# davidesantangelo/krep

Measured on NVIDIA H100. Metric: GB/s scanned (HBM-resident corpus), higher is better.
Workload: dtype u8

## Files before the change

### krep_b200/csrc/engine.cu

```cuda
#include <cub/device/device_radix_sort.cuh>
#include <algorithm>
#include <chrono>
#include <cstdarg>
#include <cstdio>
#include <cstdlib>
#include <cstring>
#include <mutex>
#include <thread>
#include "common.h"
#include "corpus.h"
#include "engine.h"

namespace kb {

static thread_local int t_err = 0;
static thread_local char t_errmsg[512] = "";

void set_error(int code, const char *fmt, ...)
{
    t_err = code;
    va_list ap;
    va_start(ap, fmt);
    vsnprintf(t_errmsg, sizeof t_errmsg, fmt, ap);
    va_end(ap);
// ... 397 lines not shown
    for (size_t i = 1; i < m; i++)
    {
        int k = pi[i - 1];
        while (k > 0 && ch(i) != ch((size_t)k)) k = pi[(size_t)k - 1];
        if (ch(i) == ch((size_t)k)) k++;
        pi[i] = k;
    }
    return pi[m - 1] == 0;
}

Plan *regex_plan_build(const search_params_t *P, std::string *why)
{
    std::string re;
    if (!regex_source(P, &re))
    {
        *why = "no pattern";
        return nullptr;
    }
    RegexDfa *D = new RegexDfa();
    if (regex_compile(re, !P->case_sensitive, D, why) != 0)
    {
        delete D;
        return nullptr;
    }
    Plan *pl = new Plan();
    pl->algo = KREP_B200_ALGO_REGEX;
    pl->is_regex = true;
    pl->case_sensitive = P->case_sensitive;
    pl->whole_word = P->whole_word ? 1 : 0;
    pl->regex = re;
    pl->rx = D;
    pl->filter_name = D->widened ? "regex-lines-widened" : "regex-lines";
    std::lock_guard<std::mutex> lp(g_plans_mu);
    g_all_plans.push_back(pl);
    return pl;
}

Plan *plan_build(const search_params_t *P, int algo, bool only_matching)
{
    if (!P) return nullptr;
    if (algo == KREP_B200_ALGO_REGEX)
    {
        std::string why;
        Plan *pl = regex_plan_build(P, &why);
        if (!pl) set_error(-3, "this regex is not run on the GPU (%s); use the host's regex_search", why.c_str());
        return pl;
    }
    Plan *pl = new Plan();
    pl->algo = algo;
    pl->case_sensitive = P->case_sensitive;
    pl->count_lines = P->count_lines_mode;
    if (algo == KREP_B200_ALGO_AC)
    {
        pl->is_ac = true;
        if (P->num_patterns > AC_MAX_PATTERNS)
        {
            set_error(-3, "too many patterns (%zu > %u)", (size_t)P->num_patterns, AC_MAX_PATTERNS);
            delete pl;
            return nullptr;
        }
        for (size_t k = 0; k < P->num_patterns; k++)
        {
            const size_t len = P->pattern_lens[k];
            if (len > 1024)
            {
                set_error(-3, "pattern %zu longer than 1024 bytes (krep.c:77)", k);
                delete pl;
                return nullptr;
            }
            pl->patterns.emplace_back(P->patterns[k] ? P->patterns[k] : "", len);
            pl->pat_lens.push_back((uint32_t)len);
        }
        pl->whole_word = P->whole_word ? 1 : 0;
        if (ac_build_tables(pl) != 0)
        {
            delete pl;
            return nullptr;
        }
        std::lock_guard<std::mutex> lp(g_plans_mu);
        g_all_plans.push_back(pl);
        return pl;
    }
    size_t m = P->pattern_len;
    if (algo == KREP_B200_ALGO_MEMCHR) m = m ? 1 : 0;
    if (m == 0 || m > 1024 || !P->pattern)
    {
        set_error(-3, "literal plan needs 1..1024 pattern bytes (got %zu)", m);
        delete pl;
        return nullptr;
    }
    pl->pattern.assign(P->pattern, m);
    pl->m = (uint32_t)m;
    pl->emit_len = (algo == KREP_B200_ALGO_MEMCHR_SHORT && only_matching) ? 1u : (uint32_t)m;
    pl->border_free = border_free(pl->pattern, pl->case_sensitive);
    pl->built_only_matching = only_matching;
    if (P->whole_word)
    {
        bool tag = pl->emit_len != pl->m;
        if (algo == KREP_B200_ALGO_AVX2 || algo == KREP_B200_ALGO_AVX512 || algo == KREP_B200_ALGO_NEON) tag = true;
        if (!tag && !pl->border_free)
            tag = algo == KREP_B200_ALGO_KMP || (algo == KREP_B200_ALGO_SSE42 && !only_matching);
        pl->whole_word = tag ? 2 : 1;
    }
    pl->h_val.resize(m);
    pl->h_msk.resize(m);
    const uint8_t *pb = (const uint8_t *)pl->pattern.data();
    for (size_t k = 0; k < m; k++)
    {
        pl->h_msk[k] = (!pl->case_sensitive && is_alpha_c(pb[k])) ? 0xDF : 0xFF;
        pl->h_val[k] = pb[k] & pl->h_msk[k];
    }
    pl->fold = pl->case_sensitive ? 0xFFFFFFFFu : 0xDFDFDFDFu;
    if (pl->emit_len >= 7)
    {
        pl->filter = FILTER_ALIGNED4;
        for (int d = 0; d < 4; d++) pl->K[d] = le32(pb + d, 4) & pl->fold;
        pl->win_mask = 0xFFFFFFFFu;
        pl->filter_name = pl->case_sensitive ? "aligned4" : "aligned4-fold";
    }
    else
    {
        pl->filter = FILTER_WINDOW4;
        const uint32_t wl = pl->emit_len < 4 ? pl->emit_len : 4;
        pl->win_mask = wl == 4 ? 0xFFFFFFFFu : ((1u << (8 * wl)) - 1);
        pl->K[0] = le32(pb, wl) & pl->fold & pl->win_mask;
        pl->filter_name = pl->case_sensitive ? "window4" : "window4-fold";
    }
    std::lock_guard<std::mutex> lp(g_plans_mu);
    g_all_plans.push_back(pl);
    return pl;
}

int launch_scan(DevCtx &E, const Plan *plan, const krep_b200_shard_t *sh, int want_positions, cudaStream_t stream, int slot,
                unsigned long long *regex_lines, bool regex_matches)
{
    if (((uintptr_t)sh->d_text & 15) != 0)
    {
        set_error(-3, "shard text pointer must be 16-byte aligned");
        return -3;
    }
    const PlanDev *pd = plan_on_device(plan, E);
    if (!pd) return -2;
    uint64_t own_end = sh->own_end < sh->avail_len ? sh->own_end : sh->avail_len;
    if (plan->is_regex)
    {
        if (regex_matches && (!plan->rx->offsets_exact || !want_positions))
        {
            set_error(-3, "regex match mode needs an offsets_exact plan and the occurrence list");
            return -3;
        }
        if (regex_matches && sh->global_offset + sh->avail_len >= REGEX_MATCH_MAX_OFFSET)
        {
            set_error(-3, "regex match offsets must stay below 2^48 bytes of global offset (key layout, csrc/common.h)");
            return -3;
        }
        RegexLaunch a;
        a.text = (const uint8_t *)sh->d_text;
        a.avail_len = sh->avail_len;
        a.own_begin = sh->own_begin;
        a.own_end = own_end;
        a.global_offset = sh->global_offset;
        a.prev_byte = sh->prev_byte;
        a.next_byte = sh->next_byte;
        a.trans = pd->d_regex;
        a.ntrans = (uint32_t)plan->rx->trans.size();
        a.nclasses = plan->rx->nclasses;
        a.start = plan->rx->start;
        a.nl_class = plan->rx->nl_class;
        a.out = E.d_list[slot];
        a.cap = want_positions ? E.key_cap : 0;
        a.counter = slot_counter(E, slot);
        a.line_count = regex_lines;
        a.matches = regex_matches ? 1u : 0u;
        a.nmtrans = (uint32_t)plan->rx->match.size();
        a.match_bol = plan->rx->match_bol;
        a.match_mid = plan->rx->match_mid;
        launch_regex(a, E.sm_count, stream);
        return 0;
    }
    if (plan->is_ac)
    {
        if (sh->global_offset + sh->avail_len >= (1ull << 40))
        {
            set_error(-3, "pattern-set shards must end below 2^40 bytes of global offset (key layout, csrc/common.h)");
            return -3;
        }
        AcLaunch a;
        a.text = (const uint8_t *)sh->d_text;
        a.avail_len = sh->avail_len;
        a.own_begin = sh->own_begin;
        a.own_end = own_end;
        a.global_offset = sh->global_offset;
        a.prev_byte = sh->prev_byte;
        a.next_byte = sh->next_byte;
        a.out = E.d_list[slot];
        a.cap = want_positions ? E.key_cap : 0;
        a.counter = slot_counter(E, slot);
        a.whole_word = plan->whole_word;
        a.want_positions = (uint32_t)want_positions;
        launch_ac(plan, pd->ac, a, E.sm_count, stream);
        return 0;
    }
    LitDevParams p;
    memset(&p, 0, sizeof p);
    p.text = (const uint8_t *)sh->d_text;
    p.avail_len = sh->avail_len;
    p.own_begin = sh->own_begin;
    p.own_end = own_end;
    p.global_offset = sh->global_offset;
    p.prev_byte = sh->prev_byte;
    p.next_byte = sh->next_byte;
    uint64_t total_groups;
    if (plan->filter == FILTER_ALIGNED4)
    {
        total_groups = sh->avail_len / 16;
        p.tail_start = total_groups ? total_groups * 16 - 3 : 0;
    }
    else
    {
        total_groups = sh->avail_len >= 20 ? (sh->avail_len - 20) / 16 + 1 : 0;
        p.tail_start = total_groups * 16;
    }
    p.group_begin = sh->own_begin / 16;
    p.group_end = (own_end + 2) / 16 + 1;
    if (p.group_end > total_groups) p.group_end = total_groups;
    if (p.group_begin > p.group_end) p.group_begin = p.group_end;
    p.m = plan->m;
    p.emit_len = plan->emit_len;
    for (int d = 0; d < 4; d++) p.K[d] = plan->K[d];
    p.fold = plan->fold;
    p.win_mask = plan->win_mask;
    p.mulc[0] = 1u << 24;
    p.mulc[1] = 1u << 16;
    p.mulc[2] = 1u << 8;
    p.pat_val = pd->d_pat_val;
    p.pat_mask = pd->d_pat_mask;
    p.out = E.d_list[slot];
    p.cap = want_positions ? E.key_cap : 0;
    p.counter = slot_counter(E, slot);
    p.whole_word = plan->whole_word;
    p.want_positions = (uint32_t)want_positions;
    launch_literal(plan, p, E.sm_count, stream);
    return 0;
}

int reset_counter(DevCtx &E, int slot, cudaStream_t stream)
{
    if (E.counter_clean[slot]) return 0;
    CK(cudaMemsetAsync(slot_counter(E, slot), 0, 64, stream));
    E.counter_clean[slot] = true;
    return 0;
}

static constexpr int FIN_THREADS = 512, FIN_SLICES = 16, FIN_KEYS = FIN_THREADS / FIN_SLICES, FIN_PIECE = 2048;

__global__ void __launch_bounds__(FIN_THREADS) k_finish(unsigned long long *counter, const uint64_t *__restrict__ keys, uint64_t cap,
                                                        uint64_t *d_pack, int want_sort)
{
    __shared__ uint64_t s_keys[FIN_PIECE];
    __shared__ unsigned long long s_cnt;
    if (threadIdx.x == 0) s_cnt = counter[0];
    __syncthreads();
    const unsigned long long cnt = s_cnt;
    if (blockIdx.x == 0 && threadIdx.x == 0) d_pack[0] = cnt;
    const bool sorting = want_sort && cnt != 0 && cnt <= PACK_KEYS && cnt <= cap;
    const uint32_t n = sorting ? (uint32_t)cnt : 0u;
    const uint32_t idx = blockIdx.x * FIN_KEYS + threadIdx.x / FIN_SLICES, slice = threadIdx.x % FIN_SLICES;
    if (blockIdx.x * FIN_KEYS < n)
    {
        const uint64_t mine = idx < n ? keys[idx] : ~0ull;
        uint32_t rank = 0;
        for (uint32_t base = 0; base < n; base += FIN_PIECE)
        {
            const uint32_t m = n - base < FIN_PIECE ? n - base : FIN_PIECE;
            for (uint32_t j = threadIdx.x; j < FIN_PIECE; j += FIN_THREADS) s_keys[j] = j < m ? keys[base + j] : ~0ull;
            __syncthreads();
            const uint32_t mr = (m + 63u) & ~63u;
#pragma unroll 8
            for (uint32_t j = slice; j < mr; j += FIN_SLICES) rank += s_keys[j] < mine ? 1u : 0u;
            __syncthreads();
        }
#pragma unroll
        for (int o = 1; o < FIN_SLICES; o <<= 1) rank += __shfl_xor_sync(0xffffffffu, rank, o);
        if (idx < n && slice == 0) d_pack[1 + rank] = mine;
    }
    __syncthreads();
    if (threadIdx.x == 0)
    {
        __threadfence();
        const unsigned long long done = atomicAdd(&counter[1], 1ULL);
        if (done == gridDim.x - 1)
        {
            counter[0] = 0;
            counter[1] = 0;
        }
    }
}

int finish_scan(DevCtx &E, int slot, int want_sort, cudaStream_t stream)
{
    k_finish<<<PACK_KEYS / FIN_KEYS, FIN_THREADS, 0, stream>>>(slot_counter(E, slot), E.d_list[slot], E.key_cap, E.d_pack[slot],
                                                                 (want_sort && E.d_list[slot]) ? 1 : 0);
    CK(cudaGetLastError());
    CK(cudaMemcpyAsync(E.h_pack[slot], E.d_pack[slot], (want_sort ? PACK_KEYS + 1 : 1) * sizeof(uint64_t), cudaMemcpyDeviceToHost, stream));
    CK(cudaEventRecord(E.ev_done[slot], stream));
    count_launch();
    E.counter_clean[slot] = true;
    return 0;
}

int sort_keys(DevCtx &E, int slot, uint64_t n, int end_bit, cudaStream_t stream, const uint64_t **sorted)
{
    *sorted = E.d_list[slot];
    if (n < 2) return 0;
    cub::DoubleBuffer<uint64_t> db(E.d_list[slot], E.d_alt);
    size_t need = 0;
    CK(cub::DeviceRadixSort::SortKeys(nullptr, need, db, (int64_t)n, 0, end_bit, stream));
    if (need > E.sort_tmp_bytes)
    {
        CK(cudaStreamSynchronize(stream));
        cudaFree(E.d_sort_tmp);
        E.d_sort_tmp = nullptr;
        E.sort_tmp_bytes = 0;
        CK(cudaMalloc(&E.d_sort_tmp, need));
        E.sort_tmp_bytes = need;
    }
    CK(cub::DeviceRadixSort::SortKeys(E.d_sort_tmp, need, db, (int64_t)n, 0, end_bit, stream));
    *sorted = db.Current();
    return 0;
}

static int bits_for(uint64_t v)
{
    int b = 1;
    while (b < 64 && (v >> b)) b++;
    return b;
}

int key_end_bit(const Plan *plan, uint64_t max_offset, bool regex_matches)
{
    const int shift = plan->is_ac ? AC_END_SHIFT : regex_matches ? REGEX_MATCH_SHIFT : LIT_TAG_BITS;
    int b = bits_for(max_offset) + shift;
    return b > 64 ? 64 : b;
}

__global__ void __launch_bounds__(256) k_line_bounds(const uint8_t *__restrict__ text, uint64_t avail, uint64_t go,
                                                     const uint64_t *__restrict__ keys, uint64_t n, int is_ac, int has_prev,
                                                     int has_next, uint64_t *__restrict__ out)
{
    const uint64_t i = ((uint64_t)blockIdx.x * blockDim.x + threadIdx.x) >> 5;
    const int lane = threadIdx.x & 31;
    if (i >= n) return;
    auto start_of = [&](uint64_t key) -> uint64_t {
        if (!is_ac) return (key >> LIT_TAG_BITS) - go;
        return (key >> AC_END_SHIFT) - (1024 - ((key >> AC_LEN_SHIFT) & 1023)) - go;
    };
    const uint64_t s = start_of(keys[i]);
    const uint64_t lb = (!is_ac && i > 0) ? start_of(keys[i - 1]) : 0;
    const uint64_t ub = (!is_ac && i + 1 < n) ? start_of(keys[i + 1]) : avail;
    uint64_t ls = (!is_ac && i > 0) ? LB_SAME_AS_PREV : (has_prev ? LB_OUTSIDE_SHARD : go);
    for (uint64_t hi = s; hi > lb;)
    {
        const uint64_t w0 = hi >= lb + 128 ? hi - 128 : lb;
        int best = -1;
#pragma unroll
        for (int k = 0; k < 4; k++)
        {
            const uint64_t p = w0 + (uint64_t)lane * 4 + k;
            if (p < hi && text[p] == '\n') best = lane * 4 + k;
        }
        best = __reduce_max_sync(0xffffffffu, best);
        if (best >= 0)
        {
            ls = go + w0 + (uint64_t)best + 1;
            break;
        }
        hi = w0;
    }
    uint64_t le = (!is_ac && i + 1 < n) ? LB_SAME_AS_NEXT : (has_next ? LB_OUTSIDE_SHARD : go + avail);
    for (uint64_t lo = s; lo < ub; lo += 128)
    {
        int best = 1 << 20;
#pragma unroll
        for (int k = 3; k >= 0; k--)
        {
            const uint64_t p = lo + (uint64_t)lane * 4 + k;
            if (p < ub && text[p] == '\n') best = lane * 4 + k;
        }
        best = __reduce_min_sync(0xffffffffu, best);
        if (best < (1 << 20))
        {
            le = go + lo + (uint64_t)best;
            break;
        }
    }
    if (lane == 0)
    {
        out[2 * i] = ls;
        out[2 * i + 1] = le;
    }
}

static int line_bounds(DevCtx &E, const Plan *plan, const krep_b200_shard_t *sh, const uint64_t *d_sorted, uint64_t n,
                       cudaStream_t stream, const uint64_t **d_bounds)
{
    *d_bounds = nullptr;
    if (n == 0) return 0;
    if (2 * n > E.bounds_cap)
    {
        CK(cudaStreamSynchronize(stream));
        cudaFree(E.d_bounds);
        E.d_bounds = nullptr;
        E.bounds_cap = 0;
        const uint64_t cap = 2 * n + n / 4 + 1024;
        CK(cudaMalloc(&E.d_bounds, cap * sizeof(uint64_t)));
        E.bounds_cap = cap;
    }
    const uint64_t threads = n * 32;
    const int has_prev = sh->prev_byte >= 0 && sh->prev_byte != '\n';
    const int has_next = sh->next_byte >= 0 && sh->next_byte != '\n';
    k_line_bounds<<<(unsigned)((threads + 255) / 256), 256, 0, stream>>>((const uint8_t *)sh->d_text, sh->avail_len, sh->global_offset,
                                                                        d_sorted, n, plan->is_ac ? 1 : 0, has_prev, has_next, E.d_bounds);
    CK(cudaGetLastError());
    count_launch();
    *d_bounds = E.d_bounds;
    return 0;
}

int scan_begin(DevCtx &E, const Plan *plan, const krep_b200_shard_t *sh, int want_positions, cudaStream_t stream, int *slot_out)
{
    if (!stream) stream = E.scan_stream;
    if (want_positions && ensure_keys(E, 1) != 0) return -2;
    const int slot = E.next_slot;
    if (E.pend[slot].active)
    {
        set_error(-3, "krep_b200_scan_shard_begin: %d scans are already in flight on device %d", SCAN_SLOTS, E.device);
        return -3;
    }
    CK(cudaStreamWaitEvent(stream, E.ev_done[slot], 0));
    if (reset_counter(E, slot, stream) != 0) return -2;
    CK(cudaEventRecord(E.ev_a[slot], stream));
    int rc = launch_scan(E, plan, sh, want_positions, stream, slot);
    if (rc != 0) return rc;
    CK(cudaEventRecord(E.ev_b[slot], stream));
    CK(cudaGetLastError());
    if (finish_scan(E, slot, want_positions, stream) != 0) return -2;
    PendingScan &P = E.pend[slot];
    P.active = true;
    P.plan = plan;
    P.shard = *sh;
    P.want_positions = want_positions;
    P.stream = stream;
    E.next_slot = (slot + 1) % SCAN_SLOTS;
    *slot_out = slot;
    return 0;
}

int scan_end(DevCtx &E, int slot, ScanOut *out)
{
    PendingScan &P = E.pend[slot];
    if (slot < 0 || slot >= SCAN_SLOTS || !P.active)
    {
        set_error(-3, "krep_b200_scan_shard_end: no scan in flight in slot %d", slot);
        return -3;
    }
    P.active = false;
    const Plan *plan = P.plan;
    const krep_b200_shard_t *sh = &P.shard;
    cudaStream_t stream = P.stream;
    reset_kernel_ms();
    for (int attempt = 0; attempt < 3; attempt++)
    {
        CK(cudaEventSynchronize(E.ev_done[slot]));
        const uint64_t cnt = E.h_pack[slot][0];
        float ms = 0.f;
        cudaEventElapsedTime(&ms, E.ev_a[slot], E.ev_b[slot]);
        add_kernel_ms(ms);
        *out = ScanOut();
        out->count = cnt;
        out->device = E.device;
        out->serial = ++E.serial;
        E.result_stream = stream;
        if (!P.want_positions) return 0;
        if (cnt <= E.key_cap)
        {
            int rc = 0;
            out->stored = cnt;
            if (cnt <= PACK_KEYS)
            {
                out->d_keys = E.d_pack[slot] + 1;
                out->h_sorted = E.h_pack[slot] + 1;
            }
            else
                rc = sort_keys(E, slot, cnt, key_end_bit(plan, sh->global_offset + sh->avail_len), stream, &out->d_keys);
            if (rc == 0 && plan->count_lines) rc = line_bounds(E, plan, sh, out->d_keys, cnt, stream, &out->d_bounds);
            return rc;
        }
        out->overflow = 1;
        for (int s2 = 0; s2 < SCAN_SLOTS; s2++)
            if (s2 != slot && E.pend[s2].active)
            {
                set_error(-3, "krep_b200_scan_shard_end: the occurrence list overflowed while another scan is in flight; end each "
                              "scan before beginning the next until the list has grown");
                return -3;
            }
        if (ensure_keys(E, cnt + cnt / 8 + 1024) != 0) return -2;
        if (reset_counter(E, slot, stream) != 0) return -2;
        CK(cudaEventRecord(E.ev_a[slot], stream));
        int rc = launch_scan(E, plan, sh, 1, stream, slot);
        if (rc != 0) return rc;
        CK(cudaEventRecord(E.ev_b[slot], stream));
        if (finish_scan(E, slot, 1, stream) != 0) return -2;
    }
    set_error(-4, "occurrence list kept overflowing");
    return -4;
}

int scan_shard(DevCtx &E, const Plan *plan, const krep_b200_shard_t *sh, int want_positions, cudaStream_t stream, ScanOut *out)
{
    int slot = 0;
    int rc = scan_begin(E, plan, sh, want_positions, stream, &slot);
    if (rc != 0) return rc;
    return scan_end(E, slot, out);
}

int fetch_keys(DevCtx &E, const ScanOut &so, const uint64_t **h)
{
    *h = nullptr;
    if (so.stored == 0) return 0;
    if (so.h_sorted)
    {
        *h = so.h_sorted;
        return 0;
    }
    if (so.stored > E.h_keys_cap)
    {
        cudaFreeHost(E.h_keys);
        E.h_keys = nullptr;
        E.h_keys_cap = 0;
        uint64_t cap = so.stored + so.stored / 4;
        if (cap < (1u << 16)) cap = 1u << 16;
        CK(cudaMallocHost(&E.h_keys, cap * sizeof(uint64_t)));
        E.h_keys_cap = cap;
    }
    cudaStream_t s = E.result_stream ? E.result_stream : E.scan_stream;
    CK(cudaMemcpyAsync(E.h_keys, so.d_keys, so.stored * sizeof(uint64_t), cudaMemcpyDeviceToHost, s));
    CK(cudaStreamSynchronize(s));
    *h = E.h_keys;
    return 0;
}

uint64_t merge_key_lists(const uint64_t *const *lists, const uint64_t *counts, uint32_t n_lists, uint64_t *dst)
{
    uint64_t total = 0;
    std::vector<uint64_t> cut;
    for (uint32_t i = 0; i < n_lists; i++)
    {
        if (counts[i] == 0) continue;
        if (dst + total != lists[i]) memmove(dst + total, lists[i], counts[i] * sizeof(uint64_t));
        cut.push_back(total);
        total += counts[i];
    }
    for (size_t i = 1; i < cut.size(); i++)
        if (dst[cut[i] - 1] > dst[cut[i]]) std::inplace_merge(dst, dst + cut[i], dst + (i + 1 < cut.size() ? cut[i + 1] : total));
    return total;
}

__global__ void __launch_bounds__(256) k_corpus(const __grid_constant__ CorpusParams c, uint8_t *dst, uint64_t global_offset,
                                                uint64_t len)
{
    const uint64_t groups = (len + 15) / 16;
    for (uint64_t g = (uint64_t)blockIdx.x * blockDim.x + threadIdx.x; g < groups; g += (uint64_t)gridDim.x * blockDim.x)
    {
        alignas(16) uint8_t b[16];
        corpus_fill16(c, global_offset + g * 16, b);
        const uint64_t off = g * 16;
        if (off + 16 <= len && (((uintptr_t)(dst + off)) & 15) == 0)
            *reinterpret_cast<uint4 *>(dst + off) = *reinterpret_cast<const uint4 *>(b);
        else
            for (int k = 0; k < 16 && off + k < len; k++) dst[off + k] = b[k];
    }
}

static int corpus_params(const krep_b200_corpus_spec_t *spec, CorpusParams *c)
{
    memset(c, 0, sizeof *c);
    c->seed = spec->seed;
    c->plant_seed = spec->plant_seed;
    c->plant_period = spec->plant_period;
    c->needle_len = spec->needle_len;
    c->flags = spec->flags;
    if (spec->needle_len > 64)
    {
        set_error(-3, "corpus needle longer than 64 bytes");
        return -3;
    }
    if (spec->plant_period && (spec->plant_period % 16 != 0 || spec->plant_period < 4ull * spec->needle_len + 32))
    {
        set_error(-3, "corpus plant_period must be a multiple of 16 and >= 4*needle_len+32");
        return -3;
    }
    if (spec->needle_len) memcpy(c->needle, spec->needle, spec->needle_len);
    return 0;
}

}

using namespace kb;

extern "C" {

int krep_b200_init(int device)
{
    g_keep_visible = true;
    warm_join();
    std::lock_guard<std::recursive_mutex> lk(engine_mutex());
    clear_error();
    if (visible_devices() == 0)
    {
        set_error(-1, "no CUDA device available; this engine has no CPU fallback");
        return -1;
    }
    if (device < 0)
    {
        device = primary_device();
        if (device < 0) return -1;
    }
    if (!ctx_get(device)) return krep_b200_last_error() ? krep_b200_last_error() : -1;
    g_primary = device;
    return 0;
}
void krep_b200_shutdown(void) { engine_shutdown(); }
int krep_b200_last_error(void) { return t_err; }
const char *krep_b200_last_error_string(void) { return t_errmsg; }
const char *krep_b200_version(void) { return "krep_b200 0.2.0 (sm_90a)"; }
int krep_b200_device_count(void)
{
    warm_join();
    return visible_devices();
}
void krep_b200_warmup(void) { warm_start(); }

float krep_b200_last_kernel_ms(void) { return t_kernel_ms; }
uint64_t krep_b200_launch_count(void) { return g_launches; }
void krep_b200_reset_launch_count(void) { g_launches = 0; }

krep_b200_plan_t *krep_b200_plan_create(const search_params_t *params, int algo)
{
    warm_join();
    std::lock_guard<std::recursive_mutex> lk(engine_mutex());
    clear_error();
    if (!params) return nullptr;
    if (visible_devices() == 0)
    {
        set_error(-1, "no CUDA device available; this engine has no CPU fallback");
        return nullptr;
    }
    return reinterpret_cast<krep_b200_plan_t *>(plan_build(params, resolve_algo(params, algo), krep_b200_get_only_matching()));
}
void krep_b200_plan_destroy(krep_b200_plan_t *plan)
{
    std::lock_guard<std::recursive_mutex> lk(engine_mutex());
    plan_free(reinterpret_cast<Plan *>(plan));
}
const char *krep_b200_plan_filter_name(const krep_b200_plan_t *plan)
{
    return plan ? reinterpret_cast<const Plan *>(plan)->filter_name.c_str() : "";
}

static DevCtx *ctx_of_pointer(const void *d_ptr)
{
    cudaPointerAttributes a;
    if (cudaPointerGetAttributes(&a, d_ptr) == cudaSuccess && a.type == cudaMemoryTypeDevice) return ctx_get(a.device);
    cudaGetLastError();
    return ctx_primary();
}

static void fill_result(const ScanOut &so, const krep_b200_shard_t *shard, int slot, krep_b200_device_result_t *out)
{
    out->count = so.count;
    out->stored = so.stored;
    out->d_keys = so.d_keys;
    out->overflow = so.overflow;
    out->text_len = shard->global_offset + shard->avail_len;
    out->d_line_bounds = so.d_bounds;
    out->device = so.device;
    out->slot = slot;
    out->serial = so.serial;
}

int krep_b200_scan_shard_begin(const krep_b200_plan_t *plan, const krep_b200_shard_t *shard, int want_positions, void *stream,
                               int *ticket)
{
    std::lock_guard<std::recursive_mutex> lk(engine_mutex());
    clear_error();
    if (!plan || !shard || !ticket)
    {
        set_error(-3, "krep_b200_scan_shard_begin: null argument");
        return -3;
    }
    DeviceGuard guard;
    DevCtx *C = ctx_of_pointer(shard->d_text);
    if (!C) return -1;
    int slot = 0;
    int rc = scan_begin(*C, reinterpret_cast<const Plan *>(plan), shard, want_positions, (cudaStream_t)stream, &slot);
    *ticket = C->device * SCAN_SLOTS + slot;
    return rc;
}

int krep_b200_scan_shard_end(int ticket, krep_b200_device_result_t *out)
{
    std::lock_guard<std::recursive_mutex> lk(engine_mutex());
    clear_error();
    if (!out || ticket < 0 || ticket >= MAX_DEV * SCAN_SLOTS)
    {
        set_error(-3, "krep_b200_scan_shard_end: bad argument");
        return -3;
    }
    DeviceGuard guard;
    DevCtx *C = ctx_get(ticket / SCAN_SLOTS);
    if (!C) return -1;
    const int slot = ticket % SCAN_SLOTS;
    const krep_b200_shard_t shard = C->pend[slot].shard;
    ScanOut so;
    int rc = scan_end(*C, slot, &so);
    fill_result(so, &shard, slot, out);
    return rc;
}

int krep_b200_scan_shard(const krep_b200_plan_t *plan, const krep_b200_shard_t *shard, int want_positions,
                         void *stream, krep_b200_device_result_t *out)
{
    int ticket = 0;
    int rc = krep_b200_scan_shard_begin(plan, shard, want_positions, stream, &ticket);
    if (rc != 0) return rc;
    if (!out)
    {
        set_error(-3, "krep_b200_scan_shard: null argument");
        return -3;
    }
    return krep_b200_scan_shard_end(ticket, out);
}

}

int kb::regex_scan_keys(DevCtx &E, const Plan *plan, const krep_b200_shard_t *shard, int mode, const char *who, uint64_t *cnt_out,
                        const uint64_t **d_sorted, uint64_t *device_lines)
{
    for (int s = 0; s < SCAN_SLOTS; s++)
        if (E.pend[s].active)
        {
            set_error(-3, "%s: a scan is in flight on device %d", who, E.device);
            return -3;
        }
    if (ensure_keys(E, 1) != 0 || (mode == 1 && ensure_line_out(E, 1) != 0)) return -2;
    unsigned long long *d_lines = mode == 1 ? (unsigned long long *)E.d_line_out : nullptr;
    const int slot = 0;
    cudaStream_t st = E.scan_stream;
    ++E.serial;
    for (int attempt = 0; attempt < 3; attempt++)
    {
        CK(cudaStreamWaitEvent(st, E.ev_done[slot], 0));
        if (reset_counter(E, slot, st) != 0) return -2;
        if (d_lines) CK(cudaMemsetAsync(d_lines, 0, sizeof(unsigned long long), st));
        int rc = launch_scan(E, plan, shard, 1, st, slot, d_lines, mode == 2);
        if (rc != 0) return rc;
        if (finish_scan(E, slot, 1, st) != 0) return -2;
        if (d_lines) CK(cudaMemcpyAsync(E.h_line_out, d_lines, sizeof(uint64_t), cudaMemcpyDeviceToHost, st));
        CK(cudaStreamSynchronize(st));
        const uint64_t cnt = E.h_pack[slot][0];
        if (cnt > E.key_cap)
        {
            if (ensure_keys(E, cnt + cnt / 8 + 1024) != 0) return -2;
            continue;
        }
        *d_sorted = E.d_pack[slot] + 1;
        if (cnt > PACK_KEYS)
        {
            rc = sort_keys(E, slot, cnt, key_end_bit(plan, shard->global_offset + shard->avail_len, mode == 2), st, d_sorted);
            if (rc != 0) return rc;
        }
        *cnt_out = cnt;
        if (device_lines) *device_lines = d_lines ? E.h_line_out[0] : 0;
        return 0;
    }
    set_error(-4, "occurrence list kept overflowing");
    return -4;
}

extern "C" {

int64_t krep_b200_regex_scan_shard_raw(const krep_b200_plan_t *plan_, const krep_b200_shard_t *shard, int mode, uint64_t *keys,
                                       uint64_t cap, uint64_t *device_lines)
{
    std::lock_guard<std::recursive_mutex> lk(engine_mutex());
    clear_error();
    const Plan *plan = reinterpret_cast<const Plan *>(plan_);
    if (!plan || !shard || (cap && !keys))
    {
        set_error(-3, "krep_b200_regex_scan_shard_raw: null argument");
        return -3;
    }
    if (!plan->is_regex || mode < 0 || mode > 2 || (mode == 1 && !plan->rx->count_exact) || (mode == 2 && !plan->rx->offsets_exact))
    {
        set_error(-3, "krep_b200_regex_scan_shard_raw: mode %d is not available for this plan", mode);
        return -3;
    }
    DeviceGuard guard;
    DevCtx *Cp = ctx_of_pointer(shard->d_text);
    if (!Cp) return -1;
    DevCtx &E = *Cp;
    uint64_t cnt = 0;
    const uint64_t *d_sorted = nullptr;
    const int rc = regex_scan_keys(E, plan, shard, mode, "krep_b200_regex_scan_shard_raw", &cnt, &d_sorted, device_lines);
    if (rc != 0) return rc;
    const uint64_t n = cnt < cap ? cnt : cap;
    if (cnt <= PACK_KEYS)
    {
        if (n) memcpy(keys, E.h_pack[0] + 1, n * sizeof(uint64_t));
    }
    else if (n)
    {
        CK(cudaMemcpyAsync(keys, d_sorted, n * sizeof(uint64_t), cudaMemcpyDeviceToHost, E.scan_stream));
        CK(cudaStreamSynchronize(E.scan_stream));
    }
    return (int64_t)cnt;
}

int krep_b200_export_keys(const krep_b200_device_result_t *dev, void *d_dst, uint64_t max_keys, void *stream)
{
    std::lock_guard<std::recursive_mutex> lk(engine_mutex());
    clear_error();
    if (!dev || !d_dst) return -3;
    const uint64_t n = dev->stored < max_keys ? dev->stored : max_keys;
    if (n == 0) return 0;
    DeviceGuard guard;
    DevCtx *C = ctx_get(dev->device);
    if (!C) return -1;
    cudaStream_t s = stream ? (cudaStream_t)stream : (C->result_stream ? C->result_stream : C->scan_stream);
    CK(cudaMemcpyAsync(d_dst, dev->d_keys, n * sizeof(uint64_t), cudaMemcpyDeviceToDevice, s));
    if (!stream) CK(cudaStreamSynchronize(s));
    return 0;
}

int krep_b200_export_packed(const krep_b200_device_result_t *dev, void *d_dst, uint64_t max_keys, void *stream)
{
    std::lock_guard<std::recursive_mutex> lk(engine_mutex());
    clear_error();
    if (!dev || !d_dst) return -3;
    DeviceGuard guard;
    DevCtx *C = ctx_get(dev->device);
    if (!C) return -1;
    cudaStream_t s = stream ? (cudaStream_t)stream : (C->result_stream ? C->result_stream : C->scan_stream);
    const uint64_t n = dev->stored < max_keys ? dev->stored : max_keys;
    if (dev->serial == C->serial && dev->stored <= PACK_KEYS && dev->slot >= 0 && dev->slot < SCAN_SLOTS)
        CK(cudaMemcpyAsync(d_dst, C->d_pack[dev->slot], (n + 1) * sizeof(uint64_t), cudaMemcpyDeviceToDevice, s));
    else
    {
        CK(cudaMemcpyAsync(d_dst, C->d_pack[dev->slot & (SCAN_SLOTS - 1)], sizeof(uint64_t), cudaMemcpyDeviceToDevice, s));
        if (n) CK(cudaMemcpyAsync((uint64_t *)d_dst + 1, dev->d_keys, n * sizeof(uint64_t), cudaMemcpyDeviceToDevice, s));
    }
    if (!stream) CK(cudaStreamSynchronize(s));
    return 0;
}

int krep_b200_export_packed_async(int ticket, void *d_dst, uint64_t max_keys)
{
    std::lock_guard<std::recursive_mutex> lk(engine_mutex());
    clear_error();
    if (!d_dst || ticket < 0 || ticket >= MAX_DEV * SCAN_SLOTS || max_keys > PACK_KEYS)
    {
        set_error(-3, "krep_b200_export_packed_async: bad argument");
        return -3;
    }
    DeviceGuard guard;
    DevCtx *C = ctx_get(ticket / SCAN_SLOTS);
    if (!C) return -1;
    const int slot = ticket % SCAN_SLOTS;
    if (!C->pend[slot].active)
    {
        set_error(-3, "krep_b200_export_packed_async: no scan in flight for this ticket");
        return -3;
    }
    cudaStream_t s = C->pend[slot].stream;
    CK(cudaStreamWaitEvent(s, C->ev_done[slot], 0));
    CK(cudaMemcpyAsync(d_dst, C->d_pack[slot], (max_keys + 1) * sizeof(uint64_t), cudaMemcpyDeviceToDevice, s));
    return 0;
}

uint64_t krep_b200_merge_keys(const uint64_t *const *lists, const uint64_t *counts, uint32_t n_lists, uint64_t *dst)
{
    if (!lists || !counts || !dst) return 0;
    return merge_key_lists(lists, counts, n_lists, dst);
}

uint64_t krep_b200_ac_key_end(uint64_t key) { return key >> AC_END_SHIFT; }
uint64_t krep_b200_ac_key_start(uint64_t key)
{
    const uint64_t len = 1024 - ((key >> AC_LEN_SHIFT) & 1023);
    return (key >> AC_END_SHIFT) - len;
}
uint32_t krep_b200_ac_key_pattern(uint64_t key) { return (uint32_t)(key & (AC_MAX_PATTERNS - 1)); }

int krep_b200_corpus_generate(const krep_b200_corpus_spec_t *spec, void *d_dst, uint64_t global_offset, uint64_t len,
                              void *stream)
{
    std::lock_guard<std::recursive_mutex> lk(engine_mutex());
    clear_error();
    DeviceGuard guard;
    DevCtx *C = ctx_of_pointer(d_dst);
    if (!C) return -1;
    CorpusParams c;
    if (corpus_params(spec, &c) != 0) return -3;
    if (global_offset % 16 != 0)
    {
        set_error(-3, "corpus global_offset must be a multiple of 16");
        return -3;
    }
    if (len == 0) return 0;
    cudaStream_t s = stream ? (cudaStream_t)stream : C->scan_stream;
    const uint64_t groups = (len + 15) / 16;
    uint64_t blocks = (groups + 255) / 256;
    const uint64_t maxb = (uint64_t)C->sm_count * 16;
    if (blocks > maxb) blocks = maxb;
    k_corpus<<<(unsigned)blocks, 256, 0, s>>>(c, (uint8_t *)d_dst, global_offset, len);
    CK(cudaGetLastError());
    if (!stream) CK(cudaStreamSynchronize(s));
    return 0;
}

int krep_b200_corpus_generate_host(const krep_b200_corpus_spec_t *spec, void *dst, uint64_t global_offset, uint64_t len)
{
    CorpusParams c;
    if (corpus_params(spec, &c) != 0) return -3;
    uint8_t *o = (uint8_t *)dst;
    uint64_t i = global_offset, end = global_offset + len;
    while (i < end)
    {
        const uint64_t g0 = i & ~15ull;
        uint8_t b[16];
        corpus_fill16(c, g0, b);
        for (uint64_t k = i - g0; k < 16 && g0 + k < end; k++) o[g0 + k - global_offset] = b[k];
        i = g0 + 16;
    }
    return 0;
}

}
```

### krep_b200/csrc/scan_literal.cu

```cuda
#include <mutex>
#include "common.h"
#include "lit_filters.cuh"

#ifndef KREP_B200_WARP_EMIT
#define KREP_B200_WARP_EMIT 1
#endif

namespace kb {

__device__ __noinline__ unsigned verify_emit(const LitDevParams &p, long long cand)
{
    const unsigned tag = verify_exact(p, cand);
    if (!tag) return 0;
    if (p.want_positions)
    {
        const unsigned long long slot = atomicAdd(p.counter, 1ULL);
        if (slot < p.cap) p.out[slot] = ((p.global_offset + (uint64_t)cand) << LIT_TAG_BITS) | (tag & 7u);
        return 0;
    }
    return 1;
}

__device__ __noinline__ unsigned slow_aligned4(const LitDevParams &p, uint64_t group, uint4 v)
{
    unsigned n = 0;
    const uint32_t w[4] = {v.x & p.fold, v.y & p.fold, v.z & p.fold, v.w & p.fold};
#pragma unroll
    for (int k = 0; k < 4; k++)
#pragma unroll
        for (int d = 0; d < 4; d++)
            if (w[k] == p.K[d]) n += verify_emit(p, (long long)(group * 16 + 4 * k) - d);
    return n;
}

template <bool WINDOW>
__device__ __noinline__ unsigned emit_warp(const LitDevParams &p, uint64_t group, uint4 v, uint32_t nx, bool mine)
{
    const uint32_t lane = threadIdx.x & 31;
    uint32_t valid = 0;
    uint64_t tags = 0;
    if (mine)
    {
        const uint32_t w[5] = {v.x, v.y, v.z, v.w, nx};
        if (WINDOW)
        {
            const uint32_t mask = p.fold & p.win_mask, k0 = p.K[0];
#pragma unroll
            for (int k = 0; k < 4; k++)
#pragma unroll
                for (int r = 0; r < 4; r++)
                {
                    const uint32_t win = r == 0 ? w[k] : __funnelshift_r(w[k], w[k + 1], 8 * r);
                    if ((win & mask) == k0)
                    {
                        const unsigned t = verify_exact(p, (long long)(group * 16 + 4 * k + r));
                        if (t)
                        {
                            valid |= 1u << (4 * k + r);
                            tags |= (uint64_t)(t & 7u) << (3 * (4 * k + r));
                        }
                    }
                }
        }
        else
        {
#pragma unroll
            for (int k = 0; k < 4; k++)
#pragma unroll
                for (int d = 0; d < 4; d++)
                    if ((w[k] & p.fold) == p.K[d])
                    {
                        const unsigned t = verify_exact(p, (long long)(group * 16 + 4 * k) - d);
                        if (t)
                        {
                            valid |= 1u << (4 * k + d);
                            tags |= (uint64_t)(t & 7u) << (3 * (4 * k + d));
                        }
                    }
        }
    }
    const uint32_t n = (uint32_t)__popc(valid);
    if (!p.want_positions) return n;
    uint32_t incl = n;
#pragma unroll
    for (int o = 1; o < 32; o <<= 1)
    {
        const uint32_t t = __shfl_up_sync(0xffffffffu, incl, o);
        if (lane >= (uint32_t)o) incl += t;
    }
    const uint32_t total = __shfl_sync(0xffffffffu, incl, 31);
    if (total == 0) return 0;
    unsigned long long base = 0;
    if (lane == 31) base = atomicAdd(p.counter, (unsigned long long)total);
    base = __shfl_sync(0xffffffffu, base, 31);
    unsigned long long slot = base + (incl - n);
    while (valid)
    {
        const uint32_t i = (uint32_t)__ffs(valid) - 1;
        valid &= valid - 1;
        const long long start = WINDOW ? (long long)(group * 16 + i) : (long long)(group * 16 + (i & ~3u)) - (long long)(i & 3u);
        if (slot < p.cap) p.out[slot] = ((p.global_offset + (uint64_t)start) << LIT_TAG_BITS) | ((tags >> (3 * i)) & 7u);
        slot++;
    }
    return 0;
}

__device__ __forceinline__ void tail_and_count(const LitDevParams &p, unsigned long long local_cnt)
{
    if (blockIdx.x == 0 && threadIdx.x < 32 && p.avail_len >= p.emit_len)
    {
        const uint64_t last = p.avail_len - p.emit_len;
        for (uint64_t s = p.tail_start + threadIdx.x; s <= last; s += 32) local_cnt += verify_emit(p, (long long)s);
    }
    if (!p.want_positions)
    {
#pragma unroll
        for (int o = 16; o > 0; o >>= 1) local_cnt += __shfl_xor_sync(0xffffffffu, local_cnt, o);
        if ((threadIdx.x & 31) == 0 && local_cnt) atomicAdd(p.counter, local_cnt);
    }
}

template <bool FOLD, int UNROLL>
__global__ void __launch_bounds__(256, 4) k_lit_aligned4(const __grid_constant__ LitDevParams p)
{
    const uint4 *__restrict__ t4 = reinterpret_cast<const uint4 *>(p.text);
    const uint32_t k0 = p.K[0], k1 = p.K[1], k2 = p.K[2], k3 = p.K[3], fold = p.fold;
    unsigned long long local_cnt = 0;
    const uint64_t tile = (uint64_t)blockDim.x * UNROLL;
    const uint64_t stride = (uint64_t)gridDim.x * tile;
    uint64_t g0 = p.group_begin + (uint64_t)blockIdx.x * tile;
    for (; g0 + tile <= p.group_end; g0 += stride)
    {
        uint4 v[UNROLL];
#pragma unroll
        for (int u = 0; u < UNROLL; u++) v[u] = ld_stream(t4 + g0 + (uint64_t)u * blockDim.x + threadIdx.x);
        bool hit = false;
#pragma unroll
        for (int u = 0; u < UNROLL; u++) hit |= hit_vec<FOLD>(v[u], fold, k0, k1, k2, k3);
#if KREP_B200_WARP_EMIT
        if (__any_sync(0xffffffffu, hit))
        {
#pragma unroll
            for (int u = 0; u < UNROLL; u++)
            {
                const bool mine = hit_vec<FOLD>(v[u], fold, k0, k1, k2, k3);
                if (__any_sync(0xffffffffu, mine))
                    local_cnt += emit_warp<false>(p, g0 + (uint64_t)u * blockDim.x + threadIdx.x, v[u], 0u, mine);
            }
        }
#else
        if (hit)
        {
#pragma unroll
            for (int u = 0; u < UNROLL; u++)
                if (hit_vec<FOLD>(v[u], fold, k0, k1, k2, k3))
                    local_cnt += slow_aligned4(p, g0 + (uint64_t)u * blockDim.x + threadIdx.x, v[u]);
        }
#endif
    }
    if (g0 < p.group_end)
    {
        for (int u = 0; u < UNROLL; u++)
        {
            const uint64_t g = g0 + (uint64_t)u * blockDim.x + threadIdx.x;
            if (g < p.group_end)
            {
                const uint4 v = ld_stream(t4 + g);
                if (hit_vec<FOLD>(v, fold, k0, k1, k2, k3)) local_cnt += slow_aligned4(p, g, v);
            }
        }
    }
    tail_and_count(p, local_cnt);
}

__device__ __noinline__ unsigned slow_window4(const LitDevParams &p, uint64_t group, uint4 v, uint32_t nx)
{
    unsigned n = 0;
    const uint32_t w[5] = {v.x, v.y, v.z, v.w, nx};
    const uint32_t mask = p.fold & p.win_mask, k0 = p.K[0];
#pragma unroll
    for (int k = 0; k < 4; k++)
#pragma unroll
        for (int r = 0; r < 4; r++)
        {
            const uint32_t win = r == 0 ? w[k] : __funnelshift_r(w[k], w[k + 1], 8 * r);
            if ((win & mask) == k0) n += verify_emit(p, (long long)(group * 16 + 4 * k + r));
        }
    return n;
}

#ifndef KREP_B200_W4_NX
#define KREP_B200_W4_NX 2
#endif
#ifndef KREP_B200_W4_WARP_EMIT
#define KREP_B200_W4_WARP_EMIT 0
#endif
#ifdef KREP_B200_W4_CS
#define WLOAD(q) ld_stream(q)
#else
#define WLOAD(q) __ldg(q)
#endif
template <bool FOLD, bool MASKED, int UNROLL>
__global__ void __launch_bounds__(256, 4) k_lit_window4(const __grid_constant__ LitDevParams p)
{
    const uint4 *__restrict__ t4 = reinterpret_cast<const uint4 *>(p.text);
    const uint32_t fold = p.fold, mask = p.win_mask, k0 = p.K[0];
    const uint32_t c1 = p.mulc[0], c2 = p.mulc[1], c3 = p.mulc[2];
    const bool lane31 = (threadIdx.x & 31) == 31;
    unsigned long long local_cnt = 0;
    const uint64_t tile = (uint64_t)blockDim.x * UNROLL;
    const uint64_t stride = (uint64_t)gridDim.x * tile;
    uint64_t g0 = p.group_begin + (uint64_t)blockIdx.x * tile;
    for (; g0 + tile <= p.group_end; g0 += stride)
    {
        uint4 v[UNROLL];
        uint32_t nx[UNROLL];
#pragma unroll
        for (int u = 0; u < UNROLL; u++)
        {
            const uint4 *q = t4 + g0 + (uint64_t)u * blockDim.x + threadIdx.x;
            v[u] = WLOAD(q);
#if KREP_B200_W4_NX == 0
            nx[u] = __ldg(reinterpret_cast<const uint32_t *>(q + 1));
#elif KREP_B200_W4_NX == 2
            nx[u] = 0u;
            asm volatile("{\n\t.reg .pred p;\n\tsetp.ne.u32 p, %2, 0;\n\t@p ld.global.nc.u32 %0, [%1];\n\t}"
                         : "+r"(nx[u])
                         : "l"(reinterpret_cast<const uint32_t *>(q + 1)), "r"((uint32_t)lane31));
#else
            nx[u] = lane31 ? __ldg(reinterpret_cast<const uint32_t *>(q + 1)) : 0u;
#endif
        }
#if KREP_B200_W4_NX != 0
#pragma unroll
        for (int u = 0; u < UNROLL; u++)
        {
            const uint32_t nb = __shfl_down_sync(0xffffffffu, v[u].x, 1);
#if KREP_B200_W4_NX == 2
            nx[u] = lane31 ? nx[u] : nb;
#else
            if (!lane31) nx[u] = nb;
#endif
        }
#endif
        uint32_t hm = 0;
#pragma unroll
        for (int u = 0; u < UNROLL; u++)
            hm |= hit_vec_w<FOLD, MASKED>(v[u], nx[u], fold, mask, k0, c1, c2, c3) ? (1u << u) : 0u;
        if constexpr (MASKED || KREP_B200_W4_WARP_EMIT)
        {
            const uint32_t anyhm = __reduce_or_sync(0xffffffffu, hm);
            if (anyhm)
            {
#pragma unroll
                for (int u = 0; u < UNROLL; u++)
                    if ((anyhm >> u) & 1u)
                        local_cnt += emit_warp<true>(p, g0 + (uint64_t)u * blockDim.x + threadIdx.x, v[u], nx[u], (hm >> u) & 1u);
            }
        }
        else if (hm)
        {
#pragma unroll
            for (int u = 0; u < UNROLL; u++)
                if ((hm >> u) & 1u) local_cnt += slow_window4(p, g0 + (uint64_t)u * blockDim.x + threadIdx.x, v[u], nx[u]);
        }
    }
    if (g0 < p.group_end)
    {
        for (int u = 0; u < UNROLL; u++)
        {
            const uint64_t g = g0 + (uint64_t)u * blockDim.x + threadIdx.x;
            if (g < p.group_end)
            {
                const uint4 v = ld_stream(t4 + g);
                const uint32_t nx = __ldg(reinterpret_cast<const uint32_t *>(t4 + g + 1));
                if (hit_vec_w<FOLD, MASKED>(v, nx, fold, mask, k0, c1, c2, c3)) local_cnt += slow_window4(p, g, v, nx);
            }
        }
    }
    tail_and_count(p, local_cnt);
}

static int g_occ[6] = {0, 0, 0, 0, 0, 0};

template <typename K>
static int occupancy(K kernel)
{
    int nb = 0;
    cudaOccupancyMaxActiveBlocksPerMultiprocessor(&nb, kernel, 256, 0);
    return nb > 0 ? nb : 1;
}

void launch_literal(const Plan *plan, const LitDevParams &p, int sm_count, cudaStream_t s)
{
    constexpr int UNROLL = 4;
    static std::once_flag once;
    std::call_once(once, [] {
        g_occ[0] = occupancy(k_lit_aligned4<false, UNROLL>);
        g_occ[1] = occupancy(k_lit_aligned4<true, UNROLL>);
        g_occ[2] = occupancy(k_lit_window4<false, false, UNROLL>);
        g_occ[3] = occupancy(k_lit_window4<true, false, UNROLL>);
        g_occ[4] = occupancy(k_lit_window4<false, true, UNROLL>);
        g_occ[5] = occupancy(k_lit_window4<true, true, UNROLL>);
    });
    const uint64_t groups = p.group_end > p.group_begin ? p.group_end - p.group_begin : 0;
    const uint64_t tile = 256ull * UNROLL;
    uint64_t tiles = (groups + tile - 1) / tile;
    if (tiles == 0) tiles = 1;
    const bool folded = plan->fold != 0xFFFFFFFFu, masked = plan->win_mask != 0xFFFFFFFFu;
    const int which = plan->filter == FILTER_WINDOW4 ? 2 + (folded ? 1 : 0) + (masked ? 2 : 0) : (folded ? 1 : 0);
    uint64_t resident = (uint64_t)sm_count * g_occ[which];
    const unsigned grid = (unsigned)(tiles < resident ? tiles : resident);
    if (which == 2)
        k_lit_window4<false, false, UNROLL><<<grid, 256, 0, s>>>(p);
    else if (which == 3)
        k_lit_window4<true, false, UNROLL><<<grid, 256, 0, s>>>(p);
    else if (which == 4)
        k_lit_window4<false, true, UNROLL><<<grid, 256, 0, s>>>(p);
    else if (which == 5)
        k_lit_window4<true, true, UNROLL><<<grid, 256, 0, s>>>(p);
    else if (which == 1)
        k_lit_aligned4<true, UNROLL><<<grid, 256, 0, s>>>(p);
    else
        k_lit_aligned4<false, UNROLL><<<grid, 256, 0, s>>>(p);
    count_launch();
}

}
```

Measured before the change: 3118.

## Give each warp a contiguous tile and take the next word from the neighbour lane

The window4 scan kernel now assigns each warp a contiguous run of 32*UNROLL groups instead of interleaving by block width. Each lane's following word comes from a rotate shuffle of the neighbour's vector, so only lane 0 issues one extra predicated load per tile instead of lane 31 issuing one per unroll step. The masked variant skips that load and does a cheap cross-boundary check on lane 31, loading the next word only on a possible partial match. Separately, the result copy to the host moves onto a separate finish stream gated by an event, and the synchronous path now waits on that event too. Together these aim to cut redundant loads and let the device-to-host copy overlap the next scan, at the cost of extra event and stream bookkeeping.

Result: no change. 3135 (median of 6 runs) (+0.6%).

```diff
diff --git a/krep_b200/csrc/engine.cu b/krep_b200/csrc/engine.cu
--- a/krep_b200/csrc/engine.cu
+++ b/krep_b200/csrc/engine.cu
@@ -723,8 +723,11 @@
     k_finish<<<PACK_KEYS / FIN_KEYS, FIN_THREADS, 0, stream>>>(slot_counter(E, slot), E.d_list[slot], E.key_cap, E.d_pack[slot],
                                                                  (want_sort && E.d_list[slot]) ? 1 : 0);
     CK(cudaGetLastError());
-    CK(cudaMemcpyAsync(E.h_pack[slot], E.d_pack[slot], (want_sort ? PACK_KEYS + 1 : 1) * sizeof(uint64_t), cudaMemcpyDeviceToHost, stream));
-    CK(cudaEventRecord(E.ev_done[slot], stream));
+    CK(cudaEventRecord(E.ev_scanned[slot], stream));
+    CK(cudaStreamWaitEvent(E.fin_stream, E.ev_scanned[slot], 0));
+    CK(cudaMemcpyAsync(E.h_pack[slot], E.d_pack[slot], (want_sort ? PACK_KEYS + 1 : 1) * sizeof(uint64_t), cudaMemcpyDeviceToHost,
+                       E.fin_stream));
+    CK(cudaEventRecord(E.ev_done[slot], E.fin_stream));
     count_launch();
     E.counter_clean[slot] = true;
     return 0;
@@ -1189,6 +1192,7 @@
         if (finish_scan(E, slot, 1, st) != 0) return -2;
         if (d_lines) CK(cudaMemcpyAsync(E.h_line_out, d_lines, sizeof(uint64_t), cudaMemcpyDeviceToHost, st));
         CK(cudaStreamSynchronize(st));
+        CK(cudaEventSynchronize(E.ev_done[slot]));
         const uint64_t cnt = E.h_pack[slot][0];
         if (cnt > E.key_cap)
         {
diff --git a/krep_b200/csrc/scan_literal.cu b/krep_b200/csrc/scan_literal.cu
--- a/krep_b200/csrc/scan_literal.cu
+++ b/krep_b200/csrc/scan_literal.cu
@@ -189,80 +189,75 @@
     return n;
 }
 
-#ifndef KREP_B200_W4_NX
-#define KREP_B200_W4_NX 2
-#endif
-#ifndef KREP_B200_W4_WARP_EMIT
-#define KREP_B200_W4_WARP_EMIT 0
-#endif
-#ifdef KREP_B200_W4_CS
-#define WLOAD(q) ld_stream(q)
-#else
-#define WLOAD(q) __ldg(q)
-#endif
+__device__ __forceinline__ uint32_t ld_next_word(const uint4 *q, bool pred)
+{
+    uint32_t w = 0u;
+    asm volatile("{\n\t.reg .pred p;\n\tsetp.ne.u32 p, %2, 0;\n\t@p ld.global.nc.u32 %0, [%1];\n\t}"
+                 : "+r"(w)
+                 : "l"(reinterpret_cast<const uint32_t *>(q)), "r"((uint32_t)pred));
+    return w;
+}
+
 template <bool FOLD, bool MASKED, int UNROLL>
 __global__ void __launch_bounds__(256, 4) k_lit_window4(const __grid_constant__ LitDevParams p)
 {
     const uint4 *__restrict__ t4 = reinterpret_cast<const uint4 *>(p.text);
     const uint32_t fold = p.fold, mask = p.win_mask, k0 = p.K[0];
     const uint32_t c1 = p.mulc[0], c2 = p.mulc[1], c3 = p.mulc[2];
-    const bool lane31 = (threadIdx.x & 31) == 31;
+    const uint32_t pm1 = mask & 0x00FFFFFFu, pm2 = mask & 0x0000FFFFu, pm3 = mask & 0x000000FFu;
+    const uint32_t lane = threadIdx.x & 31;
+    const bool lane0 = lane == 0;
+    const uint32_t src = (lane + 1) & 31;
     unsigned long long local_cnt = 0;
     const uint64_t tile = (uint64_t)blockDim.x * UNROLL;
     const uint64_t stride = (uint64_t)gridDim.x * tile;
+    const uint64_t mine = (uint64_t)(threadIdx.x >> 5) * (32 * UNROLL) + lane;
     uint64_t g0 = p.group_begin + (uint64_t)blockIdx.x * tile;
     for (; g0 + tile <= p.group_end; g0 += stride)
     {
+        const uint4 *q = t4 + g0 + mine;
         uint4 v[UNROLL];
+#pragma unroll
+        for (int u = 0; u < UNROLL; u++) v[u] = __ldg(q + 32 * u);
+        const uint32_t x = MASKED ? 0u : ld_next_word(q + 32 * UNROLL, lane0);
         uint32_t nx[UNROLL];
 #pragma unroll
         for (int u = 0; u < UNROLL; u++)
         {
-            const uint4 *q = t4 + g0 + (uint64_t)u * blockDim.x + threadIdx.x;
-            v[u] = WLOAD(q);
-#if KREP_B200_W4_NX == 0
-            nx[u] = __ldg(reinterpret_cast<const uint32_t *>(q + 1));
-#elif KREP_B200_W4_NX == 2
-            nx[u] = 0u;
-            asm volatile("{\n\t.reg .pred p;\n\tsetp.ne.u32 p, %2, 0;\n\t@p ld.global.nc.u32 %0, [%1];\n\t}"
-                         : "+r"(nx[u])
-                         : "l"(reinterpret_cast<const uint32_t *>(q + 1)), "r"((uint32_t)lane31));
-#else
-            nx[u] = lane31 ? __ldg(reinterpret_cast<const uint32_t *>(q + 1)) : 0u;
-#endif
-        }
-#if KREP_B200_W4_NX != 0
-#pragma unroll
-        for (int u = 0; u < UNROLL; u++)
-        {
-            const uint32_t nb = __shfl_down_sync(0xffffffffu, v[u].x, 1);
-#if KREP_B200_W4_NX == 2
-            nx[u] = lane31 ? nx[u] : nb;
-#else
-            if (!lane31) nx[u] = nb;
-#endif
-        }
-#endif
+            const uint32_t behind = u + 1 < UNROLL ? v[(u + 1) % UNROLL].x : x;
+            nx[u] = __shfl_sync(0xffffffffu, lane0 ? behind : v[u].x, src);
+        }
         uint32_t hm = 0;
 #pragma unroll
         for (int u = 0; u < UNROLL; u++)
             hm |= hit_vec_w<FOLD, MASKED>(v[u], nx[u], fold, mask, k0, c1, c2, c3) ? (1u << u) : 0u;
-        if constexpr (MASKED || KREP_B200_W4_WARP_EMIT)
+        if constexpr (MASKED)
+        {
+            const uint32_t w = FOLD ? v[UNROLL - 1].w & fold : v[UNROLL - 1].w;
+            const bool cross = lane == 31 && ((((w >> 8) ^ k0) & pm1) == 0 || (((w >> 16) ^ k0) & pm2) == 0 ||
+                                              (((w >> 24) ^ k0) & pm3) == 0);
+            if (cross)
+            {
+                nx[UNROLL - 1] = __ldg(reinterpret_cast<const uint32_t *>(q + 32 * (UNROLL - 1) + 1));
+                hm |= 1u << (UNROLL - 1);
+            }
+        }
+        const uint64_t gl = g0 + mine;
+        if constexpr (MASKED)
         {
             const uint32_t anyhm = __reduce_or_sync(0xffffffffu, hm);
             if (anyhm)
             {
 #pragma unroll
                 for (int u = 0; u < UNROLL; u++)
-                    if ((anyhm >> u) & 1u)
-                        local_cnt += emit_warp<true>(p, g0 + (uint64_t)u * blockDim.x + threadIdx.x, v[u], nx[u], (hm >> u) & 1u);
+                    if ((anyhm >> u) & 1u) local_cnt += emit_warp<true>(p, gl + 32 * u, v[u], nx[u], (hm >> u) & 1u);
             }
         }
         else if (hm)
         {
 #pragma unroll
             for (int u = 0; u < UNROLL; u++)
-                if ((hm >> u) & 1u) local_cnt += slow_window4(p, g0 + (uint64_t)u * blockDim.x + threadIdx.x, v[u], nx[u]);
+                if ((hm >> u) & 1u) local_cnt += slow_window4(p, gl + 32 * u, v[u], nx[u]);
         }
     }
     if (g0 < p.group_end)
```
